# zovoilis-lab/Flye

Hardware: AMD Instinct MI355X
Metric: Gbp reads overlapped/sec (higher is better)
Workload: dtype u64

## Files before the change

### flye_amd/csrc/fg_chain.hip

```cpp
#include "fg_wavesort.h"

#include <algorithm>

#define WG 256
#define I32_MIN ((i32)0x80000000)

struct ChainParams {
	int k, maxJump, minOverlap, maxOverhang;
	int checkOverhang, forceLocal;
	float minUnique;
	u32 firstId;
	u32 qFirstId;
	int onlyMaxExt;
	int keepAln;
	int ablate;
	int lazy;
	unsigned long long* lazyCnt;
};

namespace {

struct CandAcc {
	typedef int4 T;
	int4* c;
	__device__ int4 load(int i) const { return c[i]; }
	__device__ void store(int i, const int4& x) { c[i] = x; }
	__device__ bool less(const int4& a, const int4& b) const { return a.w > b.w; }
};

__device__ __forceinline__ bool overlap_test(const ChainParams& P, u32 curId, u32 extId, i32 curLen,
											 i32 extLen, i32 cb, i32 ce, i32 eb, i32 ee)
{
	const i32 curRange = ce - cb, extRange = ee - eb;
	if (curRange < P.minOverlap || extRange < P.minOverlap) return false;
	const float lengthDiff = (float)abs(curRange - extRange);
	if (lengthDiff > 0.5f * (float)min(curRange, extRange)) return false;
	if (curId == extId)
	{
		const i32 inter = min(ce, ee) - max(cb, eb);
		if (inter > curRange / 2) return false;
	}
	if (curId == (extId ^ 1u))
	{
		const i32 inter = min(ce, extLen - eb) - max(cb, extLen - ee);
		if (inter > curRange / 2) return false;
	}
	if (!P.forceLocal && P.checkOverhang)
	{
		const i32 ovh = max(min(cb, eb), min(curLen - ce, extLen - ee));
		if (ovh > P.maxOverhang) return false;
	}
	return true;
}

#define LIST_ITEMS 8
__device__ __forceinline__ void append2_offsets(const bool (&a)[LIST_ITEMS], const bool (&b)[LIST_ITEMS], u32* counts,
												u32& oA, u32& oB)
{
	__shared__ u32 wtot[2][WG / 64];
	__shared__ u32 base[2];
	const int lane = threadIdx.x & 63, wv = threadIdx.x >> 6;
	u32 cA = 0, cB = 0;
#pragma unroll
	for (int t = 0; t < LIST_ITEMS; ++t) { cA += a[t]; cB += b[t]; }
	u32 iA = cA, iB = cB;
	for (int o = 1; o < 64; o <<= 1)
	{
		const u32 x = __shfl_up(iA, o), y = __shfl_up(iB, o);
		if (lane >= o) { iA += x; iB += y; }
	}
	if (lane == 63) { wtot[0][wv] = iA; wtot[1][wv] = iB; }
	__syncthreads();
	if (threadIdx.x < 2)
	{
		u32 t = 0;
		for (int i = 0; i < WG / 64; ++i) t += wtot[threadIdx.x][i];
		base[threadIdx.x] = t ? atomicAdd(&counts[threadIdx.x], t) : 0u;
	}
	__syncthreads();
	oA = base[0] + iA - cA; oB = base[1] + iB - cB;
	for (int i = 0; i < wv; ++i) { oA += wtot[0][i]; oB += wtot[1][i]; }
}
__device__ __forceinline__ void append2_multi(const bool (&a)[LIST_ITEMS], const bool (&b)[LIST_ITEMS], u32 g0,
											  u32* listA, u32* listB, u32* counts)
{
	u32 oA, oB;
	append2_offsets(a, b, counts, oA, oB);
#pragma unroll
	for (int t = 0; t < LIST_ITEMS; ++t)
	{
		if (a[t]) listA[oA++] = g0 + (u32)t;
		if (b[t]) listB[oB++] = g0 + (u32)t;
	}
}

template <bool CLASSES>
__global__ void k_group_list(u64 nGroups, u64 nHits, const u64* __restrict__ groupStart, u32 minSize,
							 const u32* __restrict__ groupFirstCur, const u32* __restrict__ groupLastCur, i32 minOverlap,
							 u32* __restrict__ list, u32* __restrict__ listBig, u32 bigMin, u32 hugeMax, u32 mid,
							 u32* __restrict__ listFused, u32 fusedMax , u32* __restrict__ counts,
// ... 147 lines not shown

	u32* oc = gCur + g0;
	u32* oe = gExt + g0;
	const bool extSorted = extLen > curLen;
	if (inLds)
	{
		wsort::wave_mem_fence();
		if (extSorted)
		{
			bool asc = true;
			for (i32 i = lane + 1; i < n; i += 64) asc = asc && sExt[wv][i] > sExt[wv][i - 1];
			if (__builtin_amdgcn_ballot_w64(!asc))
				wsort::wave_sort<u32, unsigned short>(sExt[wv], sCur[wv], n, sPL[wv], sPR[wv], stack[wv], small[wv]);
		}
		for (i32 i = lane; i < n; i += 64) { oc[i] = sCur[wv][i]; oe[i] = sExt[wv][i]; }
	}
	else if (!extSorted)
	{
		for (i32 i = lane; i < n; i += 64) { oc[i] = hitKey.cur(g0 + i); oe[i] = hitKey.val(g0 + i); }
	}
	else
	{
		bool asc = true;
		for (i32 i = lane; i < n; i += 64)
		{
			const u32 e = hitKey.val(g0 + i);
			oc[i] = hitKey.cur(g0 + i); oe[i] = e;
			if (i > 0) asc = asc && e > hitKey.val(g0 + i - 1);
		}
		wsort::wave_mem_fence();
		if (__builtin_amdgcn_ballot_w64(!asc))
		{
			u32* aux = gAux + 4 * g0;
			wsort::wave_sort<u32, u32>(oe, oc, n, aux, aux + n, stack[wv], small[wv]);
		}
	}
}

__device__ __forceinline__ i32 wave_shr1(i32 v, i32 fill)
{
	return __builtin_amdgcn_update_dpp(fill, v, 0x138, 0xf, 0xf, false);
}
__device__ __forceinline__ i32 wave_incl_max(i32 v)
{
	v = max(v, __builtin_amdgcn_update_dpp(I32_MIN, v, 0x111, 0xf, 0xf, false));
	v = max(v, __builtin_amdgcn_update_dpp(I32_MIN, v, 0x112, 0xf, 0xf, false));
	v = max(v, __builtin_amdgcn_update_dpp(I32_MIN, v, 0x114, 0xf, 0xf, false));
	v = max(v, __builtin_amdgcn_update_dpp(I32_MIN, v, 0x118, 0xf, 0xf, false));
	v = max(v, __builtin_amdgcn_update_dpp(I32_MIN, v, 0x142, 0xa, 0xf, false));
	v = max(v, __builtin_amdgcn_update_dpp(I32_MIN, v, 0x143, 0xc, 0xf, false));
	return v;
}

#ifndef DP_WAVES
#define DP_WAVES 1
#endif
#ifndef DP_RING
#define DP_RING 256
#endif

__device__ __forceinline__ bool dp_scan_step(i32 ns, u64 mA, int rhoB, i32 firstJ, i32& maxScore, i32& maxId)
{
	const i32 exc = max(wave_incl_max(__builtin_amdgcn_update_dpp(0, ns, 0x138, 0xf, 0xf, true)), maxScore);
	const u64 updM = __builtin_amdgcn_ballot_w64(ns > exc);
	const u64 stopM = (updM & mA) | (rhoB < 64 ? (1ULL << rhoB) : 0ULL);
	const u64 lim = stopM ? (((stopM & (0 - stopM)) << 1) - 1) : ~0ULL;
	const u64 um = updM & lim;
	if (um)
	{
		const int lu = 63 - __clzll(um);
		maxScore = __builtin_amdgcn_readlane(ns, __builtin_amdgcn_readfirstlane(lu));
		maxId = firstJ - lu;
	}
	return stopM != 0;
}

__device__ __forceinline__ u32 abs_diff(i32 a, i32 b)
{
	u32 r;
	asm("v_sad_u32 %0, %1, %2, 0" : "=v"(r) : "v"(a), "v"(b));
	return r;
}

template <bool EXTS, bool WHOLE = false>
__device__ __forceinline__ void dp_group(const int k, const i32 maxJump, const i32 n, const u32* __restrict__ cur,
										 const u32* __restrict__ ext, i32* score, i32* __restrict__ back,
										 i32* ringC, i32* ringE, i32* ringS)
{
	const int lane = threadIdx.x & 63;
	const i32 negLane4 = (-1 - lane) * 4;
	const i32 FAR = -(1 << 30);
	i32 pc = FAR, pe = FAR, ps = 0;
	i32 pmv = 0x7fffffff, pmRun = I32_MIN;
	i32 ntc = lane < n ? (i32)cur[lane] : 0, nte = lane < n ? (i32)ext[lane] : 0;
	asm volatile("" : "+v"(ntc), "+v"(nte));
	for (i32 tb0 = 0; tb0 < n; tb0 += 64)
	{
		const i32 tc = ntc, te = nte;
		ntc = tb0 + 64 + lane < n ? (i32)cur[tb0 + 64 + lane] : 0;
		nte = tb0 + 64 + lane < n ? (i32)ext[tb0 + 64 + lane] : 0;
		const bool valid = tb0 + lane < n;
		const i32 pcl = __builtin_amdgcn_readlane(pc, 63), pel = __builtin_amdgcn_readlane(pe, 63),
				  psl = __builtin_amdgcn_readlane(ps, 63);
		const i32 dc0 = tc - wave_shr1(tc, pcl), de0 = te - wave_shr1(te, pel);
		const bool fast = valid && dc0 == de0 && (u32)(dc0 - 1) < (u32)(min(k, maxJump) - 1) && tb0 + lane >= 2;
		u64 headM = __builtin_amdgcn_ballot_w64(valid && !fast);
		const i32 hl = wave_incl_max(fast ? -1 : lane);
		const i32 chead = __builtin_amdgcn_ds_bpermute(max(hl, 0) << 2, tc);
		const i32 off = tc - (hl >= 0 ? chead : pcl);
		i32 ts = psl + off;
		i32 tbk = tb0 + lane - 1;
		if (tb0 == 0)
		{
			ts = lane == 0 ? 0 : ts;
			tbk = lane == 0 ? -1 : tbk;
			headM &= ~1ULL;
		}
		while (headM)
		{
			const int il = __builtin_amdgcn_readfirstlane(__ffsll((long long)headM) - 1);
			headM &= headM - 1;
			const i32 i = tb0 + il;
			const i32 cn = __builtin_amdgcn_readlane(tc, il), en = __builtin_amdgcn_readlane(te, il);
			i32 maxScore = 0, maxId = 0;
			bool done;
			{
				const bool own = lane < il;
				const i32 cp = own ? tc : pc, ep = own ? te : pe, sj = own ? ts : ps;
				const i32 dc = cn - cp, de = en - ep;
				const bool inr = max((u32)(dc - 1), (u32)(de - 1)) < (u32)(maxJump - 1);
				const i32 jd = (i32)abs_diff(dc, de);
				i32 nsRaw = sj + min(min(dc, de), k) - (jd > 100 ? 2 * jd : (jd >> 1));
				asm volatile("" : "+v"(nsRaw));
				const i32 ns = inr ? nsRaw : I32_MIN;
				const u64 inrM = __builtin_amdgcn_ballot_w64(inr);
				const u64 mB = __builtin_amdgcn_ballot_w64((EXTS ? de : dc) > maxJump);
				const u64 mAn = __builtin_amdgcn_ballot_w64(dc == de) & __builtin_amdgcn_ballot_w64(dc < k) & inrM;
				const i32 nsR = __builtin_amdgcn_ds_bpermute((il * 4 + negLane4) & 0xfc, ns);
				u64 mA = 0;
				if (mAn)
				{
					const u64 R = __brevll(mAn);
					const int sh = (64 - il) & 63;
					mA = sh ? (R >> sh) | (R << (64 - sh)) : R;
				}
				done = dp_scan_step(nsR, mA, __popcll(~mB), i - 1, maxScore, maxId);
			}
			for (i32 jb = i - 65; jb >= 0 && !done; jb -= 64)
			{
				{
					const int blk = jb >> 6;
					if (blk < 64 && __builtin_amdgcn_readlane(pmv, blk) <= maxScore - k) break;
				}
				const i32 j = jb - lane;
				i32 cp = FAR, ep = FAR, sj = 0;
				if (j >= 0)
				{
					if (WHOLE) { cp = (i32)cur[j]; ep = (i32)ext[j]; sj = score[j]; }
					else if (j >= tb0 - DP_RING)
					{
						cp = ringC[j & (DP_RING - 1)]; ep = ringE[j & (DP_RING - 1)]; sj = ringS[j & (DP_RING - 1)];
					}
					else
					{
						__builtin_amdgcn_s_waitcnt(0);
						cp = (i32)cur[j]; ep = (i32)ext[j];
						sj = __hip_atomic_load(&score[j], __ATOMIC_RELAXED, __HIP_MEMORY_SCOPE_AGENT);
					}
				}
				const i32 dc = cn - cp, de = en - ep;
				const bool inr = max((u32)(dc - 1), (u32)(de - 1)) < (u32)(maxJump - 1);
				const i32 jd = (i32)abs_diff(dc, de);
				i32 nsRaw = sj + min(min(dc, de), k) - (jd > 100 ? 2 * jd : (jd >> 1));
				asm volatile("" : "+v"(nsRaw));
				const i32 ns = inr ? nsRaw : I32_MIN;
				const u64 inrM = __builtin_amdgcn_ballot_w64(inr);
				const u64 mB = __builtin_amdgcn_ballot_w64((EXTS ? de : dc) > maxJump);
				const u64 mA = __builtin_amdgcn_ballot_w64(dc == de) & __builtin_amdgcn_ballot_w64(dc < k) & inrM;
				done = dp_scan_step(ns, mA, __popcll(~mB), jb, maxScore, maxId);
			}
			const i32 sNew = max(maxScore, k);
			ts = hl == il ? sNew + off : ts;
			tbk = lane == il ? (maxScore > k ? maxId : -1) : tbk;
		}
		asm volatile("" : "+v"(ntc), "+v"(nte));
		if (valid)
		{
			score[tb0 + lane] = ts; back[tb0 + lane] = tbk;
			if (!WHOLE) { ringC[(tb0 + lane) & (DP_RING - 1)] = tc; ringE[(tb0 + lane) & (DP_RING - 1)] = te; ringS[(tb0 + lane) & (DP_RING - 1)] = ts; }
		}
		if (WHOLE) wsort::wave_mem_fence();
		{
			const i32 tileMax = __builtin_amdgcn_readlane(wave_incl_max(valid ? ts : I32_MIN), 63);
			pmRun = max(pmRun, tileMax);
			const int t = tb0 >> 6;
			if (t < 64) pmv = lane == t ? pmRun : pmv;
		}
		pc = tc; pe = te; ps = ts;
	}
}

__global__ void __launch_bounds__(DP_WAVES * 64)
k_chain_dp(ChainParams P, const u32* __restrict__ list, u32 nList, u64 nGroups, u64 nHits,
		   const u64* __restrict__ groupStart, const u32* __restrict__ groupQuery,
		   const u32* __restrict__ query, const i32* __restrict__ len, const i32* __restrict__ qLen,
		   const uint8_t* __restrict__ groupExtSorted, const u32* __restrict__ dpSize,
		   const u32* __restrict__ gCur, const u32* __restrict__ gExt,
		   i32* __restrict__ gScore, i32* __restrict__ gBack)
{
	const u32 li = blockIdx.x * DP_WAVES + (threadIdx.x >> 6);
	if (li >= nList) return;
	const u64 g = fg_uni(list[li]);
	if (fg_uni(dpSize[g]) == 0) return;
	const u64 g0 = fg_uni(groupStart[g]);
	const u64 gend = (g + 1 < nGroups) ? fg_uni(groupStart[g + 1]) : nHits;
	const i32 n = (i32)(gend - g0);
	const bool extSorted = fg_uni((u32)groupExtSorted[g]) != 0;
	__shared__ i32 ring[DP_WAVES][3][DP_RING];
	i32* ringC = ring[threadIdx.x >> 6][0];
	i32* ringE = ring[threadIdx.x >> 6][1];
	i32* ringS = ring[threadIdx.x >> 6][2];
	if (extSorted) dp_group<true>(P.k, P.maxJump, n, gCur + g0, gExt + g0, gScore + g0, gBack + g0, ringC, ringE, ringS);
	else dp_group<false>(P.k, P.maxJump, n, gCur + g0, gExt + g0, gScore + g0, gBack + g0, ringC, ringE, ringS);
}

template <int R>
__device__ __forceinline__ i32 fast_score_order(const i32 n, const i32* score, const i32* back, u32* oval)
{
	const int lane = threadIdx.x & 63;
	u32 v[R];
	bool wide = false;
#pragma unroll
	for (int r = 0; r < R; ++r)
	{
		const i32 e = r * 64 + lane;
		const bool live = e < n && back[e] != -1;
		const i32 sc = live ? score[e] : 0;
		wide |= live && (u32)sc >= (1u << 22);
		v[r] = live ? ((u32)((1 << 22) - 1 - sc) << 10) | (u32)e : 0xFFFFFFFFu;
	}
	if (__builtin_amdgcn_ballot_w64(wide)) return -1;
#pragma unroll
	for (int k = 2; k <= 64 * R; k <<= 1)
	{
#pragma unroll
		for (int j = k >> 1; j > 0; j >>= 1)
		{
			if (j >= 64)
			{
#pragma unroll
				for (int r = 0; r < R; ++r)
				{
					const int rp = r ^ (j >> 6);
					if (rp > r)
					{
						const bool asc = ((r * 64) & k) == 0;
						const u32 lo = min(v[r], v[rp]), hi = max(v[r], v[rp]);
						v[r] = asc ? lo : hi; v[rp] = asc ? hi : lo;
					}
				}
			}
			else
			{
#pragma unroll
				for (int r = 0; r < R; ++r)
				{
					const u32 o = (u32)__shfl_xor((int)v[r], j);
					const bool asc = (((r * 64 + lane) & k) == 0);
					const bool lower = (lane & j) == 0;
					v[r] = (asc == lower) ? min(v[r], o) : max(v[r], o);
				}
			}
		}
	}
	bool tie = false;
	i32 nLive = 0;
#pragma unroll
	for (int r = 0; r < R; ++r)
	{
		u32 nx = (u32)__shfl_down((int)v[r], 1);
		const u32 first = r + 1 < R ? (u32)__builtin_amdgcn_readlane((int)v[r + 1 < R ? r + 1 : r], 0) : 0xFFFFFFFFu;
		if (lane == 63) nx = first;
		tie |= nx != 0xFFFFFFFFu && (nx >> 10) == (v[r] >> 10);
		nLive += __popcll(__builtin_amdgcn_ballot_w64(v[r] != 0xFFFFFFFFu));
	}
	if (__builtin_amdgcn_ballot_w64(tie)) return -1;
#pragma unroll
	for (int r = 0; r < R; ++r)
		if (v[r] != 0xFFFFFFFFu) oval[r * 64 + lane] = v[r] & 1023u;
	return nLive;
}


enum { LZ_ENTERED = 0, LZ_FAST, LZ_NOLIVE, LZ_TIE, LZ_ROOT, LZ_TEST, LZ_ROW = 8 };
__device__ __forceinline__ void lazy_count(const ChainParams& P, int what)
{
	if ((threadIdx.x & 63) == 0)
		atomicAdd(&P.lazyCnt[(size_t)(blockIdx.x & (FG_LAZY_STRIPES - 1)) * LZ_ROW + what], 1ULL);
}

template <bool USE_LDS, int BT_CAP>
__device__ __forceinline__ bool lazy_primary(const ChainParams& P, const i32 n, const u32 curId, const u32 extId, const i32 curLen,
											 const i32 extLen, const u32* cur, const u32* ext, const i32* score, const i32* back,
											 i32* stage, u32* ja, u32* jb, int4* cd, u32* primCountG)
{
	const int lane = threadIdx.x & 63;
	const bool staged = !USE_LDS && BT_CAP > 0 && n <= BT_CAP;
	i32 bs = I32_MIN, bi = 0;
	bool tie = false, toZero = false;
#pragma unroll 4
	for (i32 i = lane; i < n; i += 64)
	{
		i32 b, s;
		if (USE_LDS)
		{
			b = back[i]; s = score[i];
			ja[i] = b == -1 ? (u32)i << 16 : ((u32)b << 16) | 1u;
		}
		else
		{
			b = __hip_atomic_load(&back[i], __ATOMIC_RELAXED, __HIP_MEMORY_SCOPE_AGENT);
			s = __hip_atomic_load(&score[i], __ATOMIC_RELAXED, __HIP_MEMORY_SCOPE_AGENT);
			if (staged) stage[i] = b;
		}
		toZero |= b == 0;
		if (b != -1)
		{
			tie = s == bs ? true : (s > bs ? false : tie);
			bi = s > bs ? i : bi;
			bs = max(bs, s);
		}
	}
	const i32 top = __builtin_amdgcn_readlane(wave_incl_max(bs), 63);
	if (top == I32_MIN) { lazy_count(P, LZ_NOLIVE); return true; }
	const u64 topM = __builtin_amdgcn_ballot_w64(bs == top);
	if ((topM & (topM - 1)) || __builtin_amdgcn_ballot_w64(tie && bs == top)) { lazy_count(P, LZ_TIE); return false; }
	const i32 last = __builtin_amdgcn_readlane(bi, __builtin_amdgcn_readfirstlane(__ffsll((long long)topM) - 1));
	const bool anyToZero = __builtin_amdgcn_ballot_w64(toZero) != 0;
	i32 first = last, chainLength = 0;
	if (USE_LDS)
	{
		u32 *src = ja, *dst = jb;
		wsort::wave_mem_fence();
		while (true)
		{
			const u32 w = fg_uni(src[last]), a = w >> 16;
			if ((fg_uni(src[a]) >> 16) == a) { first = (i32)a; chainLength = (i32)(w & 0xffffu) + 1; break; }
			for (i32 i = lane; i <= last; i += 64)
			{
				const u32 w1 = src[i], w2 = src[w1 >> 16];
				dst[i] = (w2 & 0xffff0000u) | ((w1 + w2) & 0xffffu);
			}
			wsort::wave_mem_fence();
			u32* t = src; src = dst; dst = t;
		}
	}
	else
	{
		if (staged) wsort::wave_mem_fence();
		i32 wbase = -0x40000000, win = -1, pos = last;
		while (true)
		{
			if (pos < wbase || pos >= wbase + 64)
			{
				wbase = max(0, pos - 63);
				if (staged) win = wbase + lane < n ? stage[wbase + lane] : -1;
				else win = wbase + lane < n ? __hip_atomic_load(&back[wbase + lane], __ATOMIC_RELAXED, __HIP_MEMORY_SCOPE_AGENT) : -1;
			}
			const i32 np = __builtin_amdgcn_readlane(win, __builtin_amdgcn_readfirstlane(pos - wbase));
			first = pos;
			++chainLength;
			if (np == -1) break;
			pos = np;
		}
	}
	if (first != 0 && anyToZero) { lazy_count(P, LZ_ROOT); return false; }
	const i32 cb = (i32)cur[first], eb = (i32)ext[first];
	const i32 ce = (i32)cur[last] + P.k - 1, ee = (i32)ext[last] + P.k - 1;
	if (!overlap_test(P, curId, extId, curLen, extLen, cb, ce, eb, ee)) { lazy_count(P, LZ_TEST); return false; }
	if (lane == 0)
	{
		cd[0] = make_int4(first, last, chainLength, top - score[first] + P.k - 1);
		*primCountG = 1;
	}
	lazy_count(P, LZ_FAST);
	return true;
}

template <bool USE_LDS, int BT_CAP>
__device__ __forceinline__ void finish_group(const ChainParams& P, const i32 n, const u32 curId, const u32 extId, const i32 curLen,
											 const i32 extLen, const u32* cur, const u32* ext, i32* score, i32* back, u32* okey, u32* oval,
											 unsigned short* plLds, int* stack, int* small, i32* btLds, int4* cd, u32* primCountG)
{
	const int lane = threadIdx.x & 63;
	const int k = P.k;
	lazy_count(P, LZ_ENTERED);
	if (P.lazy && lazy_primary<USE_LDS, BT_CAP>(P, n, curId, extId, curLen, extLen, cur, ext, score, back, btLds, okey, oval, cd, primCountG))
		return;
	i32 nOrder = -1;
	if (USE_LDS && !(P.ablate & 64))
	{
		if (n <= 64) nOrder = fast_score_order<1>(n, score, back, oval);
		else if (n <= 128) nOrder = fast_score_order<2>(n, score, back, oval);
		else if (n <= 256) nOrder = fast_score_order<4>(n, score, back, oval);
	}
	const bool exact = nOrder < 0;
	if (exact)
	{
		for (i32 i = lane; i < n; i += 64) { okey[i] = (u32)(0x7fffffff - score[i]); oval[i] = (u32)i; }
		nOrder = n;
	}
	wsort::wave_mem_fence();
	if (exact && !(P.ablate & 2))
	{
		if (USE_LDS)
			wsort::wave_sort<u32, unsigned short>(okey, oval, n, plLds, plLds + n, stack, small);
		else if (BT_CAP > 0 && n <= BT_CAP)
		{
			unsigned short* pl = (unsigned short*)btLds;
			wsort::wave_sort<u32, unsigned short>(okey, oval, n, pl, pl + BT_CAP, stack, small);
		}
		else wsort::wave_sort<u32, u32>(okey, oval, n, oval + n, oval + 2 * n, stack, small);
	}

	if (P.ablate & 8) return;
	if (!USE_LDS && P.keepAln)
	{
		i32* bc = (i32*)(oval + n);
		for (i32 i = lane; i < n; i += 64) bc[i] = back[i];
		back = bc;
	}
	if (BT_CAP > 0 && n <= BT_CAP)
	{
		for (i32 i = lane; i < n; i += 64) btLds[i] = back[i];
		back = btLds;
	}
	i32 ncand = 0;
	int4 best = make_int4(0, 0, 0, 0);
	wsort::wave_mem_fence();
	i32 wbase = -0x40000000, win = -1;
	bool dirty = false;
	auto flushWin = [&]()
	{
		if (dirty)
		{
			if (wbase + lane < n) back[wbase + lane] = win;
			wsort::wave_mem_fence();
			dirty = false;
		}
	};
	auto loadWin = [&](i32 pos)
	{
		flushWin();
		wbase = max(0, pos - 63);
		if (USE_LDS || (BT_CAP > 0 && n <= BT_CAP)) win = wbase + lane < n ? back[wbase + lane] : -1;
		else win = wbase + lane < n ? __hip_atomic_load(&back[wbase + lane], __ATOMIC_RELAXED, __HIP_MEMORY_SCOPE_AGENT) : -1;
	};
	const bool inMemory = !USE_LDS && !(BT_CAP > 0 && n <= BT_CAP);
	for (i32 oi0 = 0; inMemory && oi0 < nOrder; oi0 += 64)
	{
		flushWin();
		const bool in = oi0 + lane < nOrder;
		const i32 st = in ? (i32)oval[oi0 + lane] : 0;
		i32 bk = -1;
		if (in)
		{
			if (USE_LDS || (BT_CAP > 0 && n <= BT_CAP)) bk = back[st];
			else bk = __hip_atomic_load(&back[st], __ATOMIC_RELAXED, __HIP_MEMORY_SCOPE_AGENT);
		}
		u64 m = __builtin_amdgcn_ballot_w64(bk != -1);
		while (m)
		{
			const int l = __ffsll((long long)m) - 1;
			m &= m - 1;
			const i32 start = __builtin_amdgcn_readlane(st, __builtin_amdgcn_readfirstlane(l));
			if (start < wbase || start >= wbase + 64) loadWin(start);
			if (__builtin_amdgcn_readlane(win, __builtin_amdgcn_readfirstlane(start - wbase)) == -1) continue;
			i32 firstM = 0, chainLength = 0, pos = start;
			while (true)
			{
// ... 27 lines not shown
		while (m)
		{
			const int l = __ffsll((long long)m) - 1;
			m &= m - 1;
			const i32 start = __builtin_amdgcn_readlane(st, __builtin_amdgcn_readfirstlane(l));
			if (lane == 0)
			{
				i32 firstM = 0, chainLength = 0, pos = start;
				while (pos != -1)
				{
					firstM = pos;
					++chainLength;
					const i32 np = back[pos];
					back[pos] = -1;
					pos = np;
				}
				const i32 cb = (i32)cur[firstM], eb = (i32)ext[firstM];
				const i32 ce = (i32)cur[start] + k - 1, ee = (i32)ext[start] + k - 1;
				if (overlap_test(P, curId, extId, curLen, extLen, cb, ce, eb, ee))
				{
					const int4 c4 = make_int4(firstM, start, chainLength, score[start] - score[firstM] + k - 1);
					cd[ncand] = c4;
					if (ncand == 0 || c4.w > best.w) best = c4;
					++ncand;
				}
			}
			if (m)
			{
				wsort::wave_mem_fence();
				const i32 bk2 = in ? back[st] : -1;
				m &= __builtin_amdgcn_ballot_w64(bk2 != -1);
			}
		}
	}
	wsort::wave_mem_fence();
	if (lane != 0) return;
	if (ncand == 0) return;
	if (ncand > 16)
	{
		CandAcc acc{cd};
		fgsort::sort(acc, 0, ncand, stack);
		best = cd[0];
	}
	if (P.onlyMaxExt)
	{
		cd[0] = best;
		*primCountG = 1;
		return;
	}
	if (ncand <= 16)
		for (i32 a = 1; a < ncand; ++a)
		{
			const int4 v = cd[a];
			i32 b = a - 1;
			while (b >= 0 && cd[b].w < v.w) { cd[b + 1] = cd[b]; --b; }
			cd[b + 1] = v;
		}
	i32 nprim = 0;
	for (i32 a = 0; a < ncand; ++a)
	{
		const int4 o = cd[a];
		const i32 ocb = (i32)cur[o.x], oce = (i32)cur[o.y], oeb = (i32)ext[o.x], oee = (i32)ext[o.y];
		bool contained = false;
		for (i32 b = 0; b < nprim && !contained; ++b)
		{
			const int4 pr = cd[b];
			contained = pr.w > o.w && (i32)cur[pr.x] <= ocb && oce <= (i32)cur[pr.y] &&
						(i32)ext[pr.x] <= oeb && oee <= (i32)ext[pr.y];
		}
		if (!contained) cd[nprim++] = o;
	}
	*primCountG = (u32)nprim;
}


template <int CAP, int FIN_WAVES, int BT_CAP = 0>
__global__ void __launch_bounds__(FIN_WAVES * 64)
k_chain_finish(ChainParams P, const u32* __restrict__ list, u32 nList, u64 nGroups, u64 nHits,
			   const u64* __restrict__ groupStart, const u32* __restrict__ groupQuery,
			   const u32* __restrict__ query, const i32* __restrict__ len, const i32* __restrict__ qLen,
			   const u32* __restrict__ groupExt,
			   const u32* __restrict__ gCur, const u32* __restrict__ gExt, i32* __restrict__ gScore,
			   i32* __restrict__ gBack, u32* __restrict__ gAux , int4* __restrict__ cand,
			   u32* __restrict__ primCount, const u32* __restrict__ dpSize)
{
	constexpr bool USE_LDS = CAP > 0;
	extern __shared__ __attribute__((aligned(16))) char finLds[];
	__shared__ int stack[FIN_WAVES][3 * 40];
	__shared__ int small[FIN_WAVES][3 * 8];
	__shared__ i32 btLds[FIN_WAVES][BT_CAP > 0 ? BT_CAP : 1];
	const int wv = threadIdx.x >> 6;
	const int lane = threadIdx.x & 63;
	const u32 li = blockIdx.x * FIN_WAVES + wv;
	if (li >= nList) return;
	const u64 g = fg_uni(list[li]);
	if (fg_uni(dpSize[g]) == 0) return;
	const u64 g0 = fg_uni(groupStart[g]);
	const u64 gend = (g + 1 < nGroups) ? fg_uni(groupStart[g + 1]) : nHits;
	const i32 n = (i32)(gend - g0);
	const u32 q = groupQuery[g];
	const u32* cur = gCur + g0;
	const u32* ext = gExt + g0;
	i32 *score, *back; u32 *okey, *oval;
	unsigned short* plLds = nullptr;
	if (USE_LDS)
	{
		char* base = finLds + (size_t)wv * CAP * 20;
		score = (i32*)base; back = score + CAP; okey = (u32*)(back + CAP); oval = okey + CAP;
		plLds = (unsigned short*)(oval + CAP);
		for (i32 i = lane; i < n; i += 64) { score[i] = gScore[g0 + i]; back[i] = gBack[g0 + i]; }
		wsort::wave_mem_fence();
	}
	else
	{
		score = gScore + g0; back = gBack + g0; okey = gAux + 4 * g0; oval = okey + n;
	}
	const u32 qrec = query[q];
	const u32 extId = groupExt[g];
	finish_group<USE_LDS, BT_CAP>(P, n, P.qFirstId + qrec, extId, qLen[qrec >> 1], len[(extId - P.firstId) >> 1], cur, ext, score, back,
								  okey, oval, plLds, stack[wv], small[wv], btLds[wv], cand + g0, primCount + g);
}

template <class KT>
__global__ void __launch_bounds__(64)
k_chain_small(ChainParams P, const u32* __restrict__ list, u32 nList, u64 nGroups, u64 nHits,
			  const u64* __restrict__ groupStart, const u32* __restrict__ groupQuery,
			  const u32* __restrict__ query, const i32* __restrict__ len, const i32* __restrict__ qLen,
			  HitKeyView<KT> hitKey, const u32* __restrict__ groupExt,
			  u32* __restrict__ gCur, u32* __restrict__ gExt, i32* __restrict__ gBack, int4* __restrict__ cand,
			  u32* __restrict__ dpSize, u32* __restrict__ primCount, int cap )
{
	extern __shared__ __attribute__((aligned(16))) char smallLds[];
	u32* const sCur = (u32*)smallLds; u32* const sExt = sCur + cap;
	i32* const sScore = (i32*)(sExt + cap); i32* const sBack = sScore + cap;
	u32* const sOkey = (u32*)(sBack + cap); u32* const sOval = sOkey + cap;
	unsigned short* const sP = (unsigned short*)(sOval + cap);
	__shared__ int stack[3 * 40];
	__shared__ int small[3 * 8];
	const int lane = threadIdx.x;
	const u32 li = blockIdx.x;
	if (li >= nList) return;
	const u64 g = fg_uni(list[li]);
	const u64 g0 = fg_uni(groupStart[g]);
	const u64 gend = (g + 1 < nGroups) ? fg_uni(groupStart[g + 1]) : nHits;
	const i32 n = (i32)(gend - g0);
	const u32 qrec = query[groupQuery[g]];
	const u32 extId = groupExt[g];
	const i32 curLen = qLen[qrec >> 1];
	const i32 extLen = len[(extId - P.firstId) >> 1];
	const i32 minCur = (i32)hitKey.cur(g0), maxCur = (i32)hitKey.cur(g0 + n - 1);
	u32 uniq = 0;
	i32 minExt = 0x7fffffff, maxExt = I32_MIN;
	for (i32 i = lane; i < n; i += 64)
	{
		const u32 c = hitKey.cur(g0 + i);
		const u32 pc = i ? hitKey.cur(g0 + i - 1) : 0u;
		uniq += (c != pc);
		const i32 e = (i32)hitKey.val(g0 + i);
		minExt = min(minExt, e); maxExt = max(maxExt, e);
		sCur[i] = c; sExt[i] = (u32)e;
	}
	for (int o = 32; o > 0; o >>= 1)
	{
		uniq += __shfl_xor(uniq, o);
		minExt = min(minExt, __shfl_xor(minExt, o));
		maxExt = max(maxExt, __shfl_xor(maxExt, o));
	}
	if ((float)uniq < P.minUnique) return;
	if (maxCur - minCur < P.minOverlap || maxExt - minExt < P.minOverlap) return;
	if (P.checkOverhang && !P.forceLocal)
	{
		if (min(minCur, minExt) > P.maxOverhang) return;
		if (min(curLen - maxCur, extLen - maxExt) > P.maxOverhang) return;
	}
	if (lane == 0) dpSize[g] = (u32)n;
	const bool extSorted = extLen > curLen;
	wsort::wave_mem_fence();
	if (extSorted)
	{
		bool asc = true;
		for (i32 i = lane + 1; i < n; i += 64) asc = asc && sExt[i] > sExt[i - 1];
		if (__builtin_amdgcn_ballot_w64(!asc))
			wsort::wave_sort<u32, unsigned short>(sExt, sCur, n, sP, sP + n, stack, small);
	}
	for (i32 i = lane; i < n; i += 64) { gCur[g0 + i] = sCur[i]; gExt[g0 + i] = sExt[i]; }
	wsort::wave_mem_fence();
	if (extSorted) dp_group<true, true>(P.k, P.maxJump, n, sCur, sExt, sScore, sBack, nullptr, nullptr, nullptr);
	else dp_group<false, true>(P.k, P.maxJump, n, sCur, sExt, sScore, sBack, nullptr, nullptr, nullptr);
	wsort::wave_mem_fence();
	if (P.keepAln)
		for (i32 i = lane; i < n; i += 64) gBack[g0 + i] = sBack[i];
	finish_group<true, 0>(P, n, P.qFirstId + qrec, extId, curLen, extLen, sCur, sExt, sScore, sBack, sOkey, sOval, sP, stack, small,
						  nullptr, cand + g0, primCount + g);
}

u32 fetchU32(fg_ctx* c, const u32* dptr)
{
	u32 v;
	HIP_CHECK(hipMemcpyAsync(&v, dptr, 4, hipMemcpyDeviceToHost, c->stream));
	HIP_CHECK(hipStreamSynchronize(c->stream));
	return v;
}

}

u32 fgChainSmallMax()
{
	if (getenv("FG_CHAIN_FUSED") && atoi(getenv("FG_CHAIN_FUSED")) == 0) return 0u;
	return getenv("FG_FUSED_CAP") ? (u32)std::max(64, std::min(1024, atoi(getenv("FG_FUSED_CAP")))) : (u32)FIN_CAP_S;
}

void fgChainStage(fg_ctx* c, const fg_detector_params* p, uint8_t forceLocal, u64 nGroups, u64 nHits, int keyMode,
				  int curBits)
{
	hipStream_t s = c->stream;
	ChainParams cp;
	cp.k = c->k; cp.maxJump = p->max_jump; cp.minOverlap = p->min_overlap; cp.maxOverhang = p->max_overhang;
	cp.checkOverhang = p->max_overhang > 0; cp.forceLocal = forceLocal ? 1 : 0;
	cp.minUnique = fgChainMinUnique(p);
	cp.firstId = c->firstId;
	cp.qFirstId = c->hasQ ? c->qFirstId : c->firstId;
	cp.onlyMaxExt = p->only_max_ext ? 1 : 0;
	cp.keepAln = p->keep_alignment ? 1 : 0;
	cp.ablate = getenv("FG_ABLATE") ? atoi(getenv("FG_ABLATE")) : 0;
	cp.lazy = cp.onlyMaxExt && !(getenv("FG_CHAIN_LAZY") && atoi(getenv("FG_CHAIN_LAZY")) == 0);
	cp.lazyCnt = c->dLazyCnt.p;
	if (!nGroups) return;
	const i32* qLen = c->hasQ ? c->dQLen.p : c->dLen.p;
	u32 minSize = 0;
	while ((float)minSize < cp.minUnique) ++minSize;
	if (minSize == 0) minSize = 1;
	const u32 fusedMax = fgChainSmallMax();
	const bool fused = fusedMax != 0;
	const bool classes = fusedMax >= (u32)FIN_CAP_S;
	c->dListBig.reserve((classes ? 2 : 1) * nGroups + 1); c->dListDp.reserve((classes ? 2 : 1) * nGroups + 1);
	if (!classes) c->dListSmall.reserve(nGroups + 1);
	c->dGroupExtSorted.reserve(nGroups + 1);
	c->dListCnt.reserve(4);
	const u64 hitCap = std::max<u64>(nHits, c->hitCapHint);
	c->dCur.reserve(hitCap + 16); c->dExt.reserve(hitCap + 16);
	c->dScore.reserve(hitCap + 16); c->dBack.reserve(hitCap + 16);
	c->dTmp32.reserve(4 * hitCap + 16);
	c->dCand.reserve(hitCap + 1);
	const unsigned gridG = (unsigned)((nGroups + (u64)WG * LIST_ITEMS - 1) / ((u64)WG * LIST_ITEMS));
	if (fused) c->dListFused.reserve(nGroups + 1);
	const char* hugeEnv = getenv("FG_CHAIN_HUGE_MIN");
	HIP_CHECK(hipMemsetAsync(c->dListCnt.p, 0, 16, s));
	{ ScopedK t(c->timer, "k_group_list");
	  if (classes)
		  hipLaunchKernelGGL(k_group_list<true>, gridG, WG, 0, s, nGroups, nHits, c->dGroupStart.p, minSize, c->dGroupFirstCur.p,
							 c->dGroupLastCur.p, (i32)p->min_overlap, c->dListDp.p, c->dListBig.p,
							 hugeEnv ? (u32)atoi(hugeEnv) : (u32)FIN_CAP_M, hugeEnv ? (u32)atoi(hugeEnv) : 4096u, (u32)nGroups,
							 c->dListFused.p, fusedMax, c->dListCnt.p, c->dPrimFlag.p, c->dDpSize.p);
	  else
		  hipLaunchKernelGGL(k_group_list<false>, gridG, WG, 0, s, nGroups, nHits, c->dGroupStart.p, minSize, c->dGroupFirstCur.p,
							 c->dGroupLastCur.p, (i32)p->min_overlap, c->dListSmall.p, c->dListBig.p, (u32)PREP_CAP, 0u, 0u,
							 c->dListFused.p, fusedMax, c->dListCnt.p, c->dPrimFlag.p, c->dDpSize.p); }
	u32 nPrep[4];
	c->hScalar.reserve(8);
	HIP_CHECK(hipMemcpyAsync(c->hScalar.p, c->dListCnt.p, 16, hipMemcpyDeviceToHost, s));
	HIP_CHECK(hipStreamSynchronize(s));
	memcpy(nPrep, c->hScalar.p, 16);
	const u32 nFused = fused ? nPrep[2] : 0u;
	if (!nPrep[0] && !nPrep[1] && !nPrep[3] && !nFused) return;
	const bool sideStreams = !(getenv("FG_CHAIN_STREAMS") && atoi(getenv("FG_CHAIN_STREAMS")) == 1);
	auto launchSmall = [&]()
	{
		if (!nFused) return;
		ScopedK t(c->timer, "k_chain_small");
#define SMALL_ARGS(view) cp, c->dListFused.p, nFused, nGroups, nHits, c->dGroupStart.p, c->dGroupQuery.p, c->curQuery, c->dLen.p, qLen, \
		view, c->dGroupExt.p, c->dCur.p, c->dExt.p, c->dBack.p, c->dCand.p, c->dDpSize.p, c->dPrimFlag.p, (int)fusedMax
		const size_t ldsSmall = (size_t)fusedMax * 28;
		if (keyMode == 0 && c->hitVal16)
			hipLaunchKernelGGL(k_chain_small<K32V16>, nFused, 64, ldsSmall, s, SMALL_ARGS((HitKeyView<K32V16>{c->dHitKey32.p, c->dHitVal16.p, curBits, c->firstId})));
		else if (keyMode == 0)
			hipLaunchKernelGGL(k_chain_small<u32>, nFused, 64, ldsSmall, s, SMALL_ARGS((HitKeyView<u32>{c->dHitKey32.p, c->dHitVal.p, curBits, c->firstId})));
		else if (keyMode == 1)
			hipLaunchKernelGGL(k_chain_small<PK>, nFused, 64, ldsSmall, s, SMALL_ARGS((HitKeyView<PK>{(const PK*)c->dHitKey.p, nullptr, curBits, c->firstId})));
		else
			hipLaunchKernelGGL(k_chain_small<u64>, nFused, 64, ldsSmall, s, SMALL_ARGS((HitKeyView<u64>{c->dHitKey.p, c->dHitVal.p, curBits, c->firstId})));
#undef SMALL_ARGS
	};
	auto launchPrep = [&](const u32* list, u32 nList, hipStream_t on)
	{
		ScopedK t(c->timer, "k_group_prep", on);
#define PREP_ARGS(view) cp, list, nList, nGroups, nHits, c->dGroupStart.p, c->dGroupQuery.p, c->curQuery, c->dLen.p, qLen, \
		view, c->dGroupExt.p, c->dCur.p, c->dExt.p, c->dTmp32.p, c->dDpSize.p, c->dGroupExtSorted.p
		const unsigned gridP = (nList + PREP_WAVES - 1) / PREP_WAVES;
		if (keyMode == 0 && c->hitVal16)
			hipLaunchKernelGGL(k_group_prep<K32V16>, gridP, PREP_WAVES * 64, 0, on,
							   PREP_ARGS((HitKeyView<K32V16>{c->dHitKey32.p, c->dHitVal16.p, curBits, c->firstId})));
		else if (keyMode == 0)
			hipLaunchKernelGGL(k_group_prep<u32>, gridP, PREP_WAVES * 64, 0, on,
							   PREP_ARGS((HitKeyView<u32>{c->dHitKey32.p, c->dHitVal.p, curBits, c->firstId})));
		else if (keyMode == 1)
			hipLaunchKernelGGL(k_group_prep<PK>, gridP, PREP_WAVES * 64, 0, on,
							   PREP_ARGS((HitKeyView<PK>{(const PK*)c->dHitKey.p, nullptr, curBits, c->firstId})));
		else
			hipLaunchKernelGGL(k_group_prep<u64>, gridP, PREP_WAVES * 64, 0, on,
							   PREP_ARGS((HitKeyView<u64>{c->dHitKey.p, c->dHitVal.p, curBits, c->firstId})));
#undef PREP_ARGS
	};
#define FIN_ARGS(list, n) cp, list, n, nGroups, nHits, c->dGroupStart.p, c->dGroupQuery.p, c->curQuery, c->dLen.p, \
		qLen, c->dGroupExt.p, c->dCur.p, c->dExt.p, c->dScore.p, c->dBack.p, c->dTmp32.p, c->dCand.p, c->dPrimFlag.p, c->dDpSize.p
#define DP_ARGS(list, n) cp, list, n, nGroups, nHits, c->dGroupStart.p, c->dGroupQuery.p, c->curQuery, c->dLen.p, qLen, \
		c->dGroupExtSorted.p, c->dDpSize.p, c->dCur.p, c->dExt.p, c->dScore.p, c->dBack.p
	if (classes)
	{
		const bool smallCall = (nPrep[0] + nPrep[1] + nPrep[3] + nFused) < 65536u && !getenv("FG_CHAIN_NO_SMALL_CALL");
		const u32 nMid = nPrep[0] + (smallCall ? 0u : nPrep[3]), nHuge = nPrep[1] + (smallCall ? nPrep[3] : 0u);
		const u32* listMid = c->dListDp.p + (nGroups - nPrep[0]);
		const u32* listHuge = c->dListBig.p + (nGroups - nPrep[1]);
		const bool midLds = smallCall && (!hugeEnv || (u32)atoi(hugeEnv) <= (u32)FIN_CAP_M);
		const bool side = sideStreams && (nMid || nHuge);
		hipStream_t sMid = side ? c->stream2 : s, sHuge = side ? c->stream3 : s;
		const bool split = side && !smallCall && !nHuge && !(getenv("FG_CHAIN_SPLIT") && atoi(getenv("FG_CHAIN_SPLIT")) == 0);
		const u32 nMidB = split ? nMid / 2 : 0u, nMidA = nMid - nMidB;
		auto chain = [&](const u32* list, u32 n, hipStream_t on, bool lds)
		{
			if (!n) return;
			launchPrep(list, n, on);
			{ ScopedK t(c->timer, "k_chain_dp", on);
			  hipLaunchKernelGGL(k_chain_dp, (n + DP_WAVES - 1) / DP_WAVES, DP_WAVES * 64, 0, on, DP_ARGS(list, n)); }
			if (lds)
			{
				ScopedK t(c->timer, "k_chain_finish<lds1024>", on);
				hipLaunchKernelGGL((k_chain_finish<FIN_CAP_M, 1>), n, 64, FIN_CAP_M * 20, on, FIN_ARGS(list, n));
			}
			else
			{
				ScopedK t(c->timer, "k_chain_finish<global>", on);
				hipLaunchKernelGGL((k_chain_finish<0, FIN_WAVES_G, FIN_BT_CAP>), (n + FIN_WAVES_G - 1) / FIN_WAVES_G, FIN_WAVES_G * 64, 0, on,
								   FIN_ARGS(list, n));
			}
		};
		if (side)
		{
			HIP_CHECK(hipEventRecord(c->evFork, s));
			if (nMidA) HIP_CHECK(hipStreamWaitEvent(sMid, c->evFork, 0));
			if (nHuge || nMidB) HIP_CHECK(hipStreamWaitEvent(sHuge, c->evFork, 0));
		}
		chain(listHuge, nHuge, sHuge, false);
		chain(listMid, nMidA, sMid, midLds);
		chain(listMid + nMidA, nMidB, sHuge, midLds);
		launchSmall();
		if (side)
		{
			if (nMidA)
			{
				HIP_CHECK(hipEventRecord(c->evJoin, sMid));
				HIP_CHECK(hipStreamWaitEvent(s, c->evJoin, 0));
			}
			if (nHuge || nMidB)
			{
				HIP_CHECK(hipEventRecord(c->evJoin3, sHuge));
				HIP_CHECK(hipStreamWaitEvent(s, c->evJoin3, 0));
			}
		}
		return;
	}
	launchSmall();
	if (!nPrep[0] && !nPrep[1]) return;
	{
		hipStream_t sBig = s;
		if (sideStreams && nPrep[0] && nPrep[1])
		{
			HIP_CHECK(hipEventRecord(c->evFork, s));
			HIP_CHECK(hipStreamWaitEvent(c->stream2, c->evFork, 0));
			sBig = c->stream2;
		}
		if (nPrep[1]) launchPrep(c->dListBig.p, nPrep[1], sBig);
		if (nPrep[0]) launchPrep(c->dListSmall.p, nPrep[0], s);
		if (sBig != s)
		{
			HIP_CHECK(hipEventRecord(c->evJoin, sBig));
			HIP_CHECK(hipStreamWaitEvent(s, c->evJoin, 0));
		}
	}
	HIP_CHECK(hipMemsetAsync(c->dListCnt.p, 0, 16, s));
	const bool smallCall = (nPrep[0] + nPrep[1] + nFused) < 65536u && !getenv("FG_CHAIN_NO_SMALL_CALL");
	const u32 hugeMin = hugeEnv ? (u32)atoi(hugeEnv) : (smallCall ? (u32)FIN_CAP_M : 4096u);
	{ ScopedK t(c->timer, "k_dp_list");
	  hipLaunchKernelGGL(k_dp_list, gridG, WG, 0, s, nGroups, c->dDpSize.p, hugeMin, fusedMax, c->dListSmall.p, c->dListDp.p,
						 c->dListBig.p, c->dListCnt.p); }
	u32 hc[4];
	HIP_CHECK(hipMemcpyAsync(c->hScalar.p, c->dListCnt.p, 16, hipMemcpyDeviceToHost, s));
	HIP_CHECK(hipStreamSynchronize(s));
	memcpy(hc, c->hScalar.p, 16);
	const u32* lists[3] = {c->dListSmall.p, c->dListDp.p, c->dListBig.p};
// ... 46 lines not shown
```

Measured before the change: 5.374.

## Fold lazy primary-chain reduction into DP kernel and skip finished groups

The chain DP kernel now tracks the best score, index, ties and zero-backpointer flags while it writes scores, then runs the lazy primary-chain check itself. It records per-group state flags (finished or lazy failed) in the ext-sorted byte array. The finish kernel reads these flags and skips groups already finished, or skips a repeated lazy attempt for failed ones. This removes a re-read of the score and back arrays and part of the finish-kernel work. In exchange the DP kernel carries extra registers and a tail step that could lower occupancy.

```diff
diff --git a/flye_amd/csrc/fg_chain.hip b/flye_amd/csrc/fg_chain.hip
--- a/flye_amd/csrc/fg_chain.hip
+++ b/flye_amd/csrc/fg_chain.hip
@@ -16,6 +16,12 @@
 	int ablate;
 	int lazy;
 	unsigned long long* lazyCnt;
+};
+enum { CHAIN_LAZY_ON = 1, CHAIN_LAZY_DP = 2 };
+enum {
+	GS_EXT_SORTED = 1,
+	GS_FINISHED = 2,
+	GS_LAZY_FAILED = 4
 };
 
 namespace {
@@ -329,10 +335,25 @@
 	return r;
 }
 
-template <bool EXTS, bool WHOLE = false>
+struct LazyRed {
+	i32 bs, bi;
+	bool tie, toZero;
+};
+__device__ __forceinline__ void lazy_fold(const i32 i, const i32 s, const i32 b, i32& bs, i32& bi, bool& tie, bool& toZero)
+{
+	toZero |= b == 0;
+	if (b != -1)
+	{
+		tie = s == bs ? true : (s > bs ? false : tie);
+		bi = s > bs ? i : bi;
+		bs = max(bs, s);
+	}
+}
+
+template <bool EXTS, bool WHOLE = false, bool TRACK = false>
 __device__ __forceinline__ void dp_group(const int k, const i32 maxJump, const i32 n, const u32* __restrict__ cur,
 										 const u32* __restrict__ ext, i32* score, i32* __restrict__ back,
-										 i32* ringC, i32* ringE, i32* ringS)
+										 i32* ringC, i32* ringE, i32* ringS, LazyRed* red = nullptr)
 {
 	const int lane = threadIdx.x & 63;
 	const i32 negLane4 = (-1 - lane) * 4;
@@ -435,6 +456,7 @@
 		{
 			score[tb0 + lane] = ts; back[tb0 + lane] = tbk;
 			if (!WHOLE) { ringC[(tb0 + lane) & (DP_RING - 1)] = tc; ringE[(tb0 + lane) & (DP_RING - 1)] = te; ringS[(tb0 + lane) & (DP_RING - 1)] = ts; }
+			if (TRACK) lazy_fold(tb0 + lane, ts, tbk, red->bs, red->bi, red->tie, red->toZero);
 		}
 		if (WHOLE) wsort::wave_mem_fence();
 		{
@@ -447,29 +469,6 @@
 	}
 }
 
-__global__ void __launch_bounds__(DP_WAVES * 64)
-k_chain_dp(ChainParams P, const u32* __restrict__ list, u32 nList, u64 nGroups, u64 nHits,
-		   const u64* __restrict__ groupStart, const u32* __restrict__ groupQuery,
-		   const u32* __restrict__ query, const i32* __restrict__ len, const i32* __restrict__ qLen,
-		   const uint8_t* __restrict__ groupExtSorted, const u32* __restrict__ dpSize,
-		   const u32* __restrict__ gCur, const u32* __restrict__ gExt,
-		   i32* __restrict__ gScore, i32* __restrict__ gBack)
-{
-	const u32 li = blockIdx.x * DP_WAVES + (threadIdx.x >> 6);
-	if (li >= nList) return;
-	const u64 g = fg_uni(list[li]);
-	if (fg_uni(dpSize[g]) == 0) return;
-	const u64 g0 = fg_uni(groupStart[g]);
-	const u64 gend = (g + 1 < nGroups) ? fg_uni(groupStart[g + 1]) : nHits;
-	const i32 n = (i32)(gend - g0);
-	const bool extSorted = fg_uni((u32)groupExtSorted[g]) != 0;
-	__shared__ i32 ring[DP_WAVES][3][DP_RING];
-	i32* ringC = ring[threadIdx.x >> 6][0];
-	i32* ringE = ring[threadIdx.x >> 6][1];
-	i32* ringS = ring[threadIdx.x >> 6][2];
-	if (extSorted) dp_group<true>(P.k, P.maxJump, n, gCur + g0, gExt + g0, gScore + g0, gBack + g0, ringC, ringE, ringS);
-	else dp_group<false>(P.k, P.maxJump, n, gCur + g0, gExt + g0, gScore + g0, gBack + g0, ringC, ringE, ringS);
-}
 
 template <int R>
 __device__ __forceinline__ i32 fast_score_order(const i32 n, const i32* score, const i32* back, u32* oval)
@@ -546,15 +545,17 @@
 		atomicAdd(&P.lazyCnt[(size_t)(blockIdx.x & (FG_LAZY_STRIPES - 1)) * LZ_ROW + what], 1ULL);
 }
 
-template <bool USE_LDS, int BT_CAP>
+template <bool USE_LDS, int BT_CAP, bool REDUCED = false>
 __device__ __forceinline__ bool lazy_primary(const ChainParams& P, const i32 n, const u32 curId, const u32 extId, const i32 curLen,
 											 const i32 extLen, const u32* cur, const u32* ext, const i32* score, const i32* back,
-											 i32* stage, u32* ja, u32* jb, int4* cd, u32* primCountG)
+											 i32* stage, u32* ja, u32* jb, int4* cd, u32* primCountG, const LazyRed* pre = nullptr)
 {
 	const int lane = threadIdx.x & 63;
-	const bool staged = !USE_LDS && BT_CAP > 0 && n <= BT_CAP;
+	const bool staged = !REDUCED && !USE_LDS && BT_CAP > 0 && n <= BT_CAP;
 	i32 bs = I32_MIN, bi = 0;
 	bool tie = false, toZero = false;
+	if (REDUCED) { bs = pre->bs; bi = pre->bi; tie = pre->tie; toZero = pre->toZero; }
+	else
 #pragma unroll 4
 	for (i32 i = lane; i < n; i += 64)
 	{
@@ -627,22 +628,66 @@
 	if (!overlap_test(P, curId, extId, curLen, extLen, cb, ce, eb, ee)) { lazy_count(P, LZ_TEST); return false; }
 	if (lane == 0)
 	{
-		cd[0] = make_int4(first, last, chainLength, top - score[first] + P.k - 1);
+		const i32 sFirst = USE_LDS ? score[first] : __hip_atomic_load(&score[first], __ATOMIC_RELAXED, __HIP_MEMORY_SCOPE_AGENT);
+		cd[0] = make_int4(first, last, chainLength, top - sFirst + P.k - 1);
 		*primCountG = 1;
 	}
 	lazy_count(P, LZ_FAST);
 	return true;
+}
+
+__global__ void __launch_bounds__(DP_WAVES * 64)
+k_chain_dp(ChainParams P, const u32* __restrict__ list, u32 nList, u64 nGroups, u64 nHits,
+		   const u64* __restrict__ groupStart, const u32* __restrict__ groupQuery,
+		   const u32* __restrict__ query, const i32* __restrict__ len, const i32* __restrict__ qLen,
+		   uint8_t* __restrict__ groupState, const u32* __restrict__ dpSize,
+		   const u32* __restrict__ gCur, const u32* __restrict__ gExt,
+		   i32* __restrict__ gScore, i32* __restrict__ gBack, const u32* __restrict__ groupExt, int4* __restrict__ cand, u32* __restrict__ primCount)
+{
+	const u32 li = blockIdx.x * DP_WAVES + (threadIdx.x >> 6);
+	if (li >= nList) return;
+	const u64 g = fg_uni(list[li]);
+	if (fg_uni(dpSize[g]) == 0) return;
+	const u64 g0 = fg_uni(groupStart[g]);
+	const u64 gend = (g + 1 < nGroups) ? fg_uni(groupStart[g + 1]) : nHits;
+	const i32 n = (i32)(gend - g0);
+	const bool extSorted = (fg_uni((u32)groupState[g]) & GS_EXT_SORTED) != 0;
+	const bool lazyHere = (P.lazy & CHAIN_LAZY_DP) != 0;
+	u32 curId = 0, extId = 0;
+	i32 curLen = 0, extLen = 0;
+	if (lazyHere)
+	{
+		const u32 qrec = fg_uni(query[fg_uni(groupQuery[g])]);
+		extId = fg_uni(groupExt[g]);
+		curId = P.qFirstId + qrec;
+		curLen = fg_uni(qLen[qrec >> 1]);
+		extLen = fg_uni(len[(extId - P.firstId) >> 1]);
+	}
+	__shared__ i32 ring[DP_WAVES][3][DP_RING];
+	i32* ringC = ring[threadIdx.x >> 6][0];
+	i32* ringE = ring[threadIdx.x >> 6][1];
+	i32* ringS = ring[threadIdx.x >> 6][2];
+	LazyRed red = {I32_MIN, 0, false, false};
+	if (extSorted) dp_group<true, false, true>(P.k, P.maxJump, n, gCur + g0, gExt + g0, gScore + g0, gBack + g0, ringC, ringE, ringS, &red);
+	else dp_group<false, false, true>(P.k, P.maxJump, n, gCur + g0, gExt + g0, gScore + g0, gBack + g0, ringC, ringE, ringS, &red);
+	if (!lazyHere) return;
+	__builtin_amdgcn_s_waitcnt(0);
+	lazy_count(P, LZ_ENTERED);
+	const bool fin = lazy_primary<false, 0, true>(P, n, curId, extId, curLen, extLen, gCur + g0, gExt + g0, gScore + g0, gBack + g0,
+												  nullptr, nullptr, nullptr, cand + g0, primCount + g, &red);
+	if ((threadIdx.x & 63) == 0) groupState[g] = (uint8_t)((extSorted ? GS_EXT_SORTED : 0) | (fin ? GS_FINISHED : GS_LAZY_FAILED));
 }
 
 template <bool USE_LDS, int BT_CAP>
 __device__ __forceinline__ void finish_group(const ChainParams& P, const i32 n, const u32 curId, const u32 extId, const i32 curLen,
 											 const i32 extLen, const u32* cur, const u32* ext, i32* score, i32* back, u32* okey, u32* oval,
-											 unsigned short* plLds, int* stack, int* small, i32* btLds, int4* cd, u32* primCountG)
+											 unsigned short* plLds, int* stack, int* small, i32* btLds, int4* cd, u32* primCountG,
+											 const bool dpTried = false )
 {
 	const int lane = threadIdx.x & 63;
 	const int k = P.k;
-	lazy_count(P, LZ_ENTERED);
-	if (P.lazy && lazy_primary<USE_LDS, BT_CAP>(P, n, curId, extId, curLen, extLen, cur, ext, score, back, btLds, okey, oval, cd, primCountG))
+	if (!dpTried) lazy_count(P, LZ_ENTERED);
+	if (!dpTried && P.lazy && lazy_primary<USE_LDS, BT_CAP>(P, n, curId, extId, curLen, extLen, cur, ext, score, back, btLds, okey, oval, cd, primCountG))
 		return;
 	i32 nOrder = -1;
 	if (USE_LDS && !(P.ablate & 64))
@@ -836,7 +881,7 @@
 			   const u32* __restrict__ groupExt,
 			   const u32* __restrict__ gCur, const u32* __restrict__ gExt, i32* __restrict__ gScore,
 			   i32* __restrict__ gBack, u32* __restrict__ gAux , int4* __restrict__ cand,
-			   u32* __restrict__ primCount, const u32* __restrict__ dpSize)
+			   u32* __restrict__ primCount, const u32* __restrict__ dpSize, const uint8_t* __restrict__ groupState)
 {
 	constexpr bool USE_LDS = CAP > 0;
 	extern __shared__ __attribute__((aligned(16))) char finLds[];
@@ -849,6 +894,8 @@
 	if (li >= nList) return;
 	const u64 g = fg_uni(list[li]);
 	if (fg_uni(dpSize[g]) == 0) return;
+	const u32 state = fg_uni((u32)groupState[g]);
+	if (state & GS_FINISHED) return;
 	const u64 g0 = fg_uni(groupStart[g]);
 	const u64 gend = (g + 1 < nGroups) ? fg_uni(groupStart[g + 1]) : nHits;
 	const i32 n = (i32)(gend - g0);
@@ -872,7 +919,7 @@
 	const u32 qrec = query[q];
 	const u32 extId = groupExt[g];
 	finish_group<USE_LDS, BT_CAP>(P, n, P.qFirstId + qrec, extId, qLen[qrec >> 1], len[(extId - P.firstId) >> 1], cur, ext, score, back,
-								  okey, oval, plLds, stack[wv], small[wv], btLds[wv], cand + g0, primCount + g);
+								  okey, oval, plLds, stack[wv], small[wv], btLds[wv], cand + g0, primCount + g, (state & GS_LAZY_FAILED) != 0);
 }
 
 template <class KT>
@@ -977,7 +1024,8 @@
 	cp.onlyMaxExt = p->only_max_ext ? 1 : 0;
 	cp.keepAln = p->keep_alignment ? 1 : 0;
 	cp.ablate = getenv("FG_ABLATE") ? atoi(getenv("FG_ABLATE")) : 0;
-	cp.lazy = cp.onlyMaxExt && !(getenv("FG_CHAIN_LAZY") && atoi(getenv("FG_CHAIN_LAZY")) == 0);
+	cp.lazy = cp.onlyMaxExt && !(getenv("FG_CHAIN_LAZY") && atoi(getenv("FG_CHAIN_LAZY")) == 0) ? CHAIN_LAZY_ON : 0;
+	if (cp.lazy && !(getenv("FG_CHAIN_DP_LAZY") && atoi(getenv("FG_CHAIN_DP_LAZY")) == 0)) cp.lazy |= CHAIN_LAZY_DP;
 	cp.lazyCnt = c->dLazyCnt.p;
 	if (!nGroups) return;
 	const i32* qLen = c->hasQ ? c->dQLen.p : c->dLen.p;
@@ -1056,9 +1104,10 @@
 #undef PREP_ARGS
 	};
 #define FIN_ARGS(list, n) cp, list, n, nGroups, nHits, c->dGroupStart.p, c->dGroupQuery.p, c->curQuery, c->dLen.p, \
-		qLen, c->dGroupExt.p, c->dCur.p, c->dExt.p, c->dScore.p, c->dBack.p, c->dTmp32.p, c->dCand.p, c->dPrimFlag.p, c->dDpSize.p
+		qLen, c->dGroupExt.p, c->dCur.p, c->dExt.p, c->dScore.p, c->dBack.p, c->dTmp32.p, c->dCand.p, c->dPrimFlag.p, c->dDpSize.p, \
+		c->dGroupExtSorted.p
 #define DP_ARGS(list, n) cp, list, n, nGroups, nHits, c->dGroupStart.p, c->dGroupQuery.p, c->curQuery, c->dLen.p, qLen, \
-		c->dGroupExtSorted.p, c->dDpSize.p, c->dCur.p, c->dExt.p, c->dScore.p, c->dBack.p
+		c->dGroupExtSorted.p, c->dDpSize.p, c->dCur.p, c->dExt.p, c->dScore.p, c->dBack.p, c->dGroupExt.p, c->dCand.p, c->dPrimFlag.p
 	if (classes)
 	{
 		const bool smallCall = (nPrep[0] + nPrep[1] + nPrep[3] + nFused) < 65536u && !getenv("FG_CHAIN_NO_SMALL_CALL");
```

Result: no change. 5.369 (-0.1%).
